# imazen/image-webp

Measured on AMD Instinct MI355X. Metric: 1920x1080 lossy encodes/s (Q75, method 4), higher is better.
Workload: dtype int32; 1 GPU; encode_frame_lossy 1920x1080 RGBA Q75 m4; device_batch=1024, distinct_frames=4, mbs_per_frame=8160, parallelism=frames sharded over 1 GPU(s), steps_pipelined=True, pipeline_lanes=2

## Files before the change

image-webp_amd/csrc/zw_enc_kernels.hip:

```cpp
#include "zw_dev.h"

#include <type_traits>

#include "zw_enc_rows.h"

#ifdef ZW_NW
#define ZW_NW1 ZW_NW
#define ZW_NW2 ZW_NW
#endif
#ifndef ZW_NW1
#define ZW_NW1 12
#endif
#ifndef ZW_NW2
#define ZW_NW2 12
#endif
#define NW_MAX (ZW_NW1 > ZW_NW2 ? ZW_NW1 : ZW_NW2)
#ifndef ZW_DYN_PRIO
#define ZW_DYN_PRIO 1
#endif
#ifndef ZW_DYN_PRIO1
#define ZW_DYN_PRIO1 2
#endif
#ifndef ZW_P1_LUMA_MAX
#define ZW_P1_LUMA_MAX 3
#endif
#ifndef ZW_CHAIN_PRIO
#define ZW_CHAIN_PRIO 3
#endif
#ifndef ZW_LUMA_PRIO
#define ZW_LUMA_PRIO 0
#endif
#ifndef ZW_UVQ_CHAIN_ROWS
#define ZW_UVQ_CHAIN_ROWS 1
#endif
#ifndef ZW_UVQ_CHAIN_BATCH
#define ZW_UVQ_CHAIN_BATCH 0
#endif
#ifndef ZW_PAIR_UNROLL
#define ZW_PAIR_UNROLL 1
#endif
#ifndef ZW_FETCH_AHEAD
#define ZW_FETCH_AHEAD (PASS == 2)
#endif
#ifndef ZW_AN4_GPW
#define ZW_AN4_GPW 1
#endif

template <int PASS> struct PassShape {
    static constexpr int NW = PASS == 1 ? ZW_NW1 : ZW_NW2;
    static constexpr int WG = NW * 64;
};

__device__ __forceinline__ int rgb_y(const uint8_t* p)
{
    return (16839 * p[0] + 33059 * p[1] + 6420 * p[2] + (1 << 15) + (16 << 16)) >> 16;
}
__device__ __forceinline__ int rgb_u(const uint8_t* p) { return -9719 * p[0] - 19081 * p[1] + 28800 * p[2] + (128 << 16); }
// ... 478 lines not shown
        uint32_t t01 = cnt[0] + cnt[1], t23 = cnt[2] + cnt[3];
#define GETP(a, b) ((a) + (b) == 0 ? 255 : (uint8_t)((255 * (a) + ((a) + (b)) / 2) / ((a) + (b))))
        P.seg_probs[0] = GETP(t01, t23);
        P.seg_probs[1] = GETP(cnt[0], cnt[1]);
        P.seg_probs[2] = GETP(cnt[2], cnt[3]);
#undef GETP
        P.seg_update_map = P.seg_probs[0] != 255 || P.seg_probs[1] != 255 || P.seg_probs[2] != 255;
        P.seg_enabled = 1;
    }
    params[f] = P;
    uint4* Hz = (uint4*)(histo + (size_t)f * 256);
    for (int i = 0; i < 64; i++) Hz[i] = make_uint4(0u, 0u, 0u, 0u);
}

struct EncArgs {
    const uint8_t *Y, *U, *V;
    const uint8_t* alpha;
    const ZwFrameParams* params;
    const ZwLevelCosts* lcost;
    int8_t* derr;
    ZwMbOut* out;
    uint8_t *ry, *ru, *rv;
    size_t ysz, csz;
    int mbw, mbh, pass;
    int* dbg;
    uint8_t* rows;
    uint32_t* sizes;
    int nframes;
};

struct MbLds {
    uint8_t sy[256], su[64], sv[64];
    uint8_t ws[17 * ZW_BPS];
    uint8_t left_y[20], left_u[12], left_v[12], left_c[12];
    int8_t left_derr[4];
    uint8_t modes[16];
    int16_t lev[25][16];
};

struct WaveLds {
    MbLds mb;
    uint8_t cu[9 * ZW_BPS], cv[9 * ZW_BPS];
    uint32_t uvc[64][8];
    int dc[64];
    int y2d[64];
    int y2cost[4];
    int V[2][40];
    int nzt[4], nzl[4];
    int misc[16];
    uint32_t pst[2][4];
    uint8_t win_y[32], win_u[8], win_v[8], win_c[12];
    int8_t win_d[4];
#ifdef ZW_PHASE_PROF
    unsigned long long ph[24];
#endif
};


struct Ctx {
    const EncArgs* a;
    const ZwFrameParams* P;
    int method;
    const ZwSegment* S;
    const ZwSegment* Sl;
    const LdsTables* T;
    WaveLds* W;
    MbLds* M;
    uint8_t *top_y, *top_u, *top_v, *top_c;
    int8_t* top_derr;
    const uint8_t *srcY, *srcU, *srcV;
    const uint8_t *sY, *sU, *sV;
    int ys, cs;
    int mbx, mby, lane, seg;
    int f;
    int oy, oc, ocx, od;
};

__device__ void build_luma_border(const Ctx& C, int part = 2)
{
    uint8_t* ws = C.M->ws;
    const int l = C.lane;
    const int mbw = C.a->mbw;
    const bool want = part == 2 || (part == 0 ? (l < 17 || l >= 32) : (l >= 17 && l < 32));
    if (!want) {
    } else if (l < 32) {
        int v;
        if (l == 0) v = C.mby == 0 ? 127 : (C.mbx == 0 ? 129 : C.M->left_y[0]);
        else if (C.mby == 0) v = 127;
        else if (l <= 16) v = C.top_y[C.oy + l - 1];
        else if (C.mbx == mbw - 1) v = C.top_y[C.oy + 15];
        else v = C.top_y[C.oy + l - 1];
        ws[l] = (uint8_t)v;
        if (l >= 17 && l < 21) {
            ws[4 * ZW_BPS + l] = (uint8_t)v;
            ws[8 * ZW_BPS + l] = (uint8_t)v;
            ws[12 * ZW_BPS + l] = (uint8_t)v;
        }
    } else if (l < 48) {
        int i = l - 32;
        ws[(i + 1) * ZW_BPS] = C.mbx == 0 ? 129 : C.M->left_y[1 + i];
    }
    wsync();
}

__device__ void build_chroma_border(const Ctx& C)
{
    const int l = C.lane;
// ... 66 lines not shown
        const int d = wht_g(c[0], b);
        const int t = b > 0;
        const int ay = (int)((__umul24((uint32_t)iabs(d), S.y2.iq[t]) + S.y2.bias[t]) >> 17);
        const int qy = d < 0 ? -ay : ay;
        y2cost = (int)rcost_g<0, PASS == 2>(qy, b, 0, 1, T);
        dq[0] = iwht_g(m24(qy, (int)S.y2.q[t]), b);
    }
    idct16(dq);
    int rec[16], sse = 0, flat = 1;
    const int s00 = C.sY[0];
#pragma unroll
    for (int k = 0; k < 16; k++) {
        rec[k] = clamp255(pr[k] + dq[k]);
        const int d = src[k] - rec[k];
        sse += m24(d, d);
        flat &= src[k] == s00;
    }
    int td = iabs(ttransform_diff_pk(rec, src)) >> 5;
    sse = red16(sse);
    td = red16(td);
    cost = red16(cost);
    nzac = red16(nzac);
    flat = red16(flat);
    const int srcflat = __builtin_amdgcn_readlane(flat, 0) == 16;
    cost += y2cost;
    int sd = S.tlambda > 0 ? ((int)S.tlambda * td + 128) >> 8 : 0;
    int dfin = sse;
    if (srcflat && nzac == 0) {
        dfin = sse * 2;
        sd = sd * 2;
    }
    const int mcost = sel4(m, d_FIXED_COSTS_I16[0], d_FIXED_COSTS_I16[1], d_FIXED_COSTS_I16[2], d_FIXED_COSTS_I16[3]) + cost;
    const int dist = dfin + sd;
    long long brd = 0x7fffffffffffffffLL, bfin = 0;
    int bm = 0;
#pragma unroll
    for (int mm = 0; mm < 4; mm++) {
        const long long mc = __builtin_amdgcn_readlane(mcost, mm * 16);
        const long long dd = 256LL * __builtin_amdgcn_readlane(dist, mm * 16);
        const long long r_m = mc * (long long)S.l_i16 + dd;
        const long long f_m = mc * (long long)S.l_mode + dd;
        const int avail = mm == 0 || (mm == 1 && above) || (mm == 2 && left) || (mm == 3 && above && left);
        if (avail && r_m < brd) {
            brd = r_m;
            bfin = f_m;
            bm = mm;
        }
    }
    best_mode = bm;
    best_score = bfin < 0 ? 0ull : (unsigned long long)bfin;
}

#ifdef ZW_PHASE_PROF
__device__ unsigned long long zw_phase_cycles_dev[2][24];
__device__ unsigned long long zw_wave_cycles_dev[2][16][24];
#define PH_START() long long ph_t_ = clock64()
#define PH_RESET() (ph_t_ = clock64())
#define PH_MARK(k) PH_MARK_L(k, lane, PASS)
#define PH_MARK_L(k, ln, ps)                                                        \
    do {                                                                            \
        const long long n_ = clock64();                                             \
        if ((ln) == 0) C.W->ph[k] += (unsigned long long)(n_ - ph_t_);               \
        ph_t_ = n_;                                                                 \
    } while (0)
extern "C" int zw_wave_cycles(unsigned long long* out, int reset)
{
    if (hipMemcpyFromSymbol(out, HIP_SYMBOL(zw_wave_cycles_dev), sizeof(zw_wave_cycles_dev)) != hipSuccess) return -1;
    if (reset) {
        static unsigned long long z[2][16][24];
        if (hipMemcpyToSymbol(HIP_SYMBOL(zw_wave_cycles_dev), z, sizeof z) != hipSuccess) return -1;
    }
    return 0;
}
extern "C" int zw_phase_cycles(unsigned long long* out, int reset)
{
    if (hipMemcpyFromSymbol(out, HIP_SYMBOL(zw_phase_cycles_dev), sizeof(zw_phase_cycles_dev)) != hipSuccess) return -1;
    if (reset) {
        static unsigned long long z[2][24];
        if (hipMemcpyToSymbol(HIP_SYMBOL(zw_phase_cycles_dev), z, sizeof z) != hipSuccess) return -1;
    }
    return 0;
}
#define PH_COUNT(k) \
    do {                \
        if (C.lane == 0) C.W->ph[k] += 1; \
    } while (0)
#elif defined(ZW_ASM_MARKS)
#define PH_COUNT(k) (void)0
#define PH_START() asm volatile("; ZWMARK start" ::: "memory")
#define PH_RESET() (void)0
#define PH_MARK(k) asm volatile("; ZWMARK " #k ::: "memory")
#define PH_MARK_L(k, ln, ps) asm volatile("; ZWMARK " #k ::: "memory")
#else
#define PH_COUNT(k) (void)0
#define PH_START() (void)0
#define PH_RESET() (void)0
#define PH_MARK(k) (void)0
#define PH_MARK_L(k, ln, ps) (void)0
#endif

template <int NB>
__device__ __forceinline__ void i4_values_n(const Ctx& C, const int* x0, const int* y0)
{
    WaveLds* W = C.W;
    const uint8_t* ws = C.M->ws;
    const int l = C.lane;
    const int t = (int)(l >= 13) + (int)(l >= 24) + (int)(l >= 36) + (int)(l >= 37);
    const int k = min(l - 13 * (int)(l >= 13) - 11 * (int)(l >= 24), 12);
    const int t3 = (int)(t == 3), t4 = (int)(t >= 4), t12 = (int)(t == 1 || t == 2);
    const int ka = k + t3 * (11 - k) + t4 * (1 - k);
    const int kb = k + t12 + t3 * (12 - k) - t4 * k;
    const int kc = min(k + 2 * (int)(t == 1), 12);
    const int wb = 2 * (int)(t == 1) + (int)(t == 2) + 3 * (t3 + t4);
    const int wc = (int)(t == 1);
    const int sh = (int)(t != 0) + (int)(t != 0 && t != 2);
    const int oa = csel(ka < 4, -ka * ZW_BPS, ka - 4 - 4 * ZW_BPS);
    const int ob = csel(kb < 4, -kb * ZW_BPS, kb - 4 - 4 * ZW_BPS);
    const int oc = csel(kc < 4, -kc * ZW_BPS, kc - 4 - 4 * ZW_BPS);
    const bool dcl = l < 4 || (l >= 5 && l < 9);
    int v[NB], ea[NB];
#pragma unroll
    for (int h = 0; h < NB; h++) {
        const int rowL = (y0[h] + 3) * ZW_BPS + x0[h] - 1;
        ea[h] = ws[rowL + oa];
        const int eb = ws[rowL + ob], ec = ws[rowL + oc];
        v[h] = (ea[h] + wb * eb + wc * ec + ((1 << sh) >> 1)) >> sh;
    }
#pragma unroll
    for (int h = 0; h < NB; h++) {
        const int dsum = red16(dcl ? ea[h] : 0);
        if (l < 38) W->V[h][l] = v[h];
// ... 1135 lines not shown
        for (int i = 0; i < 16; i++) {
            const int sby = i >> 2, sbx = i & 3, x0 = sbx * 4 + 1, y0 = sby * 4 + 1;
            const int bm = C.M->modes[i];
            i4_values(C, x0, y0);
            const int k = l & 15;
            const int pk = i4_pred_at(W->V[0], i4_src_index(C.T, bm, k), W->V[0][5 + (k & 3)] - W->V[0][4]);
            const int svk = C.sY[(sby * 4 + (k >> 2)) * 16 + sbx * 4 + (k & 3)];
            const int ck = fdct_g(svk - pk, k);
            const int ctx0 = min(left_nz[sby] + top_nz[sbx], 2);
            if (C.a->dbg && C.a->pass == 2 && l < 16) {
                int* d = C.a->dbg + (((size_t)C.f * C.a->mbw * C.a->mbh + (size_t)C.mby * C.a->mbw + C.mbx) * 16 + i) * 34;
                d[k] = ck;
                d[16 + k] = pk;
                if (k == 0) {
                    d[32] = ctx0;
                    d[33] = bm;
                }
            }
            const int qs = quantz(ck, S.y1.iq[k > 0], S.y1.bias[k > 0]);
            const int snz = gmask(qs != 0) != 0;
            int dqk, nzq;
            if (trel) {
                const int cn = gget(ck, zz_of(k));
                int lvn;
                nzq = trellis_g<0>(cn, k, S.y1, S.sharpen, S.lt_i4, C.T, 3, ctx0, lvn);
                if (l < 16) C.M->lev[i][k] = (int16_t)lvn;
                dqk = m24(gget(lvn, izz_of(k)), (int)S.y1.q[k > 0]);
            } else {
                if (l < 16) C.M->lev[i][izz_of(k)] = (int16_t)qs;
                nzq = snz;
                dqk = m24(qs, (int)S.y1.q[k > 0]);
            }
            const int rk = idct_g(dqk, k);
            if (l < 16) C.M->ws[(y0 + (k >> 2)) * ZW_BPS + x0 + (k & 3)] = (uint8_t)clamp255(pk + rk);
            wsync();
            if (l == 0) {
                W->misc[1] = nzq;
                W->misc[2] = snz;
            }
            wsync();
            const int nz = W->misc[1];
            anynz |= W->misc[2];
            top_nz[sbx] = nz;
            left_nz[sby] = nz;
            y_nz_out[i] = nz;
            wsync();
        }
        if (l < 16) C.M->lev[16][l] = 0;
        wsync();
        PH_MARK_L(15, l, 0);
        PH_COUNT(7);
    }
    return anynz;
}

__device__ int final_chroma(const Ctx& C, int mode, int8_t* top_derr, int uv_nz[8])
{
    WaveLds* W = C.W;
    const ZwSegment& S = *C.S;
    const int l = C.lane;
    const int h = l >> 5, b = l & 7, pl = b >> 2, bx = b & 1, by = (b >> 1) & 1;
    const bool act = (l & 31) < 8;
    int cf[2][4];
    uint32_t p01[2], p32[2];
    {
        const uint32_t* e = W->uvc[h * 32 + mode * 8 + b];
#pragma unroll
        for (int c = 0; c < 2; c++) {
            cf[c][0] = lo16(e[2 * c]);
            cf[c][1] = hi16(e[2 * c]);
            cf[c][2] = lo16(e[2 * c + 1]);
            cf[c][3] = hi16(e[2 * c + 1]);
        }
        p01[0] = e[4];
        p32[0] = e[5];
        p01[1] = e[6];
        p32[1] = e[7];
    }
    {
        const int q = (int)S.uv.q[0];
        const uint32_t iq = S.uv.iq[0], bias = S.uv.bias[0];
        const uint32_t zt = S.uv.zthresh[0];
        int dcs[8];
#pragma unroll
        for (int k = 0; k < 8; k++) dcs[k] = __builtin_amdgcn_readlane(cf[0][0], k);
        auto diffuse = [&](int& dc, int te, int le) -> int {
            dc += (7 * te + 8 * le) >> 3;
            const int sign = dc < 0;
            const uint32_t a = (uint32_t)(sign ? -dc : dc);
            const int level = a > zt ? (int)((a * iq + bias) >> 17) : 0;
            const int err = (int)a - level * q;
            const int se = sign ? -err : err;
            const int v = se >> 1;
            return (int)(int8_t)(v < -127 ? -127 : (v > 127 ? 127 : v));
        };
#pragma unroll
        for (int ch = 0; ch < 2; ch++) {
            int8_t* top = top_derr + ch * 2;
            int8_t* lft = C.M->left_derr + ch * 2;
            const int t0 = __builtin_amdgcn_readfirstlane((int)top[0]), t1 = __builtin_amdgcn_readfirstlane((int)top[1]);
            const int l0 = __builtin_amdgcn_readfirstlane((int)lft[0]), l1 = __builtin_amdgcn_readfirstlane((int)lft[1]);
            int* d = dcs + ch * 4;
            const int e0 = diffuse(d[0], t0, l0);
            const int e1 = diffuse(d[1], t1, e0);
            const int e2 = diffuse(d[2], e0, l1);
            const int e3 = diffuse(d[3], e1, e2);
// ... 554 lines not shown
            (&Tf->lc[0][0][0][0])[i] = a.lcost ? (&a.lcost[ff].lc[0][0][0][0])[i] : 0;
        for (int i = threadIdx.x; i < 96; i += WG) {
            (&Tf->eob[0][0][0])[i] = a.lcost ? (&a.lcost[ff].eob[0][0][0])[i] : 0;
            (&Tf->init[0][0][0])[i] = a.lcost ? (&a.lcost[ff].init[0][0][0])[i] : 0;
        }
        for (int i = threadIdx.x; i < 4 * 8 * 3 * 11; i += WG) (&Tf->probs[0][0][0][0])[i] = (&Pf->probs[0][0][0][0])[i];
        static_assert(sizeof(ZwSegment) % 4 == 0, "segment copy by dwords");
        for (int i = threadIdx.x; i < (int)(4 * sizeof(ZwSegment) / 4); i += WG)
            ((uint32_t*)Sf)[i] = ((const uint32_t*)Pf->seg)[i];
        for (int i = threadIdx.x; i < 256; i += WG) lut[i] = Pf->seg_enabled ? Pf->seg_map_lut[i] : 0;
        load_static_tables(Tf, threadIdx.x, WG, &Pf->probs[0][0][0][0]);
        if (!ROWS || chain_wg) {
            uint8_t* ty = top_y + L.sy * fr;
            uint8_t* tu = top_u + L.su * fr;
            uint8_t* tv = top_v + L.sv * fr;
            uint8_t* tcx = top_c + L.sc * fr;
            int8_t* td = top_derr + L.sd * fr;
            if (!ROWS) {
                for (int i = threadIdx.x; i < mbw * 16 + 48; i += WG) ty[i] = 127;
                for (int i = threadIdx.x; i < mbw * 12; i += WG) tcx[i] = 0;
            }
            for (int i = threadIdx.x; i < mbw * 8 + 48; i += WG) {
                tu[i] = 127;
                tv[i] = 127;
            }
            for (int i = threadIdx.x; i < mbw * 4; i += WG) td[i] = PASS == 2 ? a.derr[(size_t)ff * mbw * 4 + i] : 0;
        }
    }
    if (threadIdx.x < NW) progress[threadIdx.x] = -1;
    if (threadIdx.x < 2) xflag[threadIdx.x] = 0;
    if (ROWS && lane < 12) W->win_c[lane] = 0;
    __syncthreads();

    Ctx C;
    C.a = &a;
    C.P = P;
    C.T = T;
    C.W = W;
    C.M = &W->mb;
    C.lane = lane;
    C.f = f;
    C.Sl = Sl;
    C.method = __builtin_amdgcn_readfirstlane(P->method);
    C.top_y = top_y;
    C.top_u = top_u;
    C.top_v = top_v;
    C.top_c = top_c;
    C.top_derr = top_derr;
    C.oy = C.oc = C.ocx = C.od = 0;
    const bool trel = PASS == 2 && __builtin_amdgcn_readfirstlane(P->do_trellis);
    const bool keep_i4 = !trel && (PASS == 1 || a.dbg == nullptr);
    const size_t nmb = (size_t)mbw * mbh;
#ifdef ZW_PHASE_PROF
    if (lane < 24) W->ph[lane] = 0;
    wsync();
    auto ph_flush = [&]() {
        if (lane < 24) atomicAdd(&zw_phase_cycles_dev[PASS - 1][lane], W->ph[lane]);
        if (lane < 24) atomicAdd(&zw_wave_cycles_dev[PASS - 1][wv][lane], W->ph[lane]);
    };
#else
    auto ph_flush = []() {};
#endif

    if (chain_wg) {
        __builtin_amdgcn_s_setprio(ZW_CHAIN_PRIO);
        const int cfr = PAIR ? wv : 0;
        const bool has_chain = !PAIR || cfr < nf;
        const int fc = f + (has_chain ? cfr : 0);
        const uint8_t* const lutc = seg_lut + L.sL * cfr;
        int8_t* const tdc = top_derr + L.sd * cfr;
        if (PAIR) {
            C.f = fc;
            C.P = a.params + fc;
            C.T = (const LdsTables*)((const uint8_t*)T + L.sT * cfr);
            C.Sl = (const ZwSegment*)((const uint8_t*)Sl + L.sS * cfr);
            C.top_u = top_u + L.su * cfr;
            C.top_v = top_v + L.sv * cfr;
            C.top_derr = tdc;
            C.method = __builtin_amdgcn_readfirstlane(C.P->method);
        }
        if (lane < 4) C.M->left_derr[lane] = 0;
        if (NCH == 2 && !PAIR) {
            const int pl = wv;
            UvQ U;
            U.pl = pl;
            U.w = W->cu;
            U.sp = C.M->su;
            U.top = pl ? top_v : top_u;
            U.left = C.M->left_u;
            const uint8_t* const P0 = (pl ? a.V : a.U) + (size_t)f * a.csz;
            const int cs = mbw * 8;
            auto fetch_uv = [&](int mbx, int mby) {
                MbFetch r;
                r.y = lane < 16 ? *(const uint32_t*)(P0 + (size_t)(mby * 8 + (lane >> 1)) * cs + mbx * 8 + (lane & 1) * 4)
                                : 0u;
                r.c = 0;
                r.alpha = a.alpha[(size_t)f * nmb + (size_t)mby * mbw + mbx];
                return r;
            };
            C.ys = mbw * 16;
            C.cs = cs;
            MbFetch nx = fetch_uv(0, 0);
            int seq = 0;
            for (int mby = 0; mby < mbh; mby++) {
                if (lane < 12) C.M->left_u[lane] = 129;
                wsync();
                for (int mbx = 0; mbx < mbw; mbx++) {
                    PH_START();
                    const int lane = opaque_lane(threadIdx.x & 63);
                    C.lane = lane;
                    const MbFetch cur = nx;
// ... 32 lines not shown
                C.M->left_v[lane] = 129;
            }
            wsync();
            for (int mbx = 0; mbx < mbw; mbx++) {
                PH_START();
                const int lane = opaque_lane(threadIdx.x & 63);
                C.lane = lane;
                const MbFetch cur = nx;
                if (mbx + 1 < mbw) nx = fetch_mb(&a, fc, lane, mbx + 1, mby);
                else if (mby + 1 < mbh) nx = fetch_mb(&a, fc, lane, 0, mby + 1);
                setup_ctx(C, &a, lutc, W, mbx, mby, cur);
                C.oc = mbx * 8;
                C.ocx = mbx * 12;
                build_chroma_border(C);
                const int cm = pick_uv<PASS>(C);
                PH_MARK(8);
                int uvnz[8];
                final_chroma(C, cm, tdc + mbx * 4, uvnz);
                PH_MARK(9);
                store_chroma_borders(C);
                ZwMbOut* o = a.out + (size_t)fc * nmb + (size_t)mby * mbw + mbx;
                if (lane == 0) o->chroma_mode = (uint8_t)cm;
                write_levels(C, 17, 8, false);
                wsync();
            }
        }
        for (int i = lane; has_chain && i < mbw * 4; i += 64) a.derr[(size_t)fc * mbw * 4 + i] = tdc[i];
        if (!PAIR) {
            ph_flush();
            return;
        }
        C.f = f;
        C.P = P;
        C.T = T;
        C.Sl = Sl;
        C.top_u = top_u;
        C.top_v = top_v;
        C.top_derr = top_derr;
        C.method = __builtin_amdgcn_readfirstlane(P->method);
    }

    if (PASS == 1) __builtin_amdgcn_s_setprio(ZW_LUMA_PRIO);
    using RS = RowSchedule<PASS, ROWS, NW, NCH>;
    constexpr bool skip_mode = RS::skip_mode;
    constexpr int nrw = RS::nrw;
    const int rw = ROWS ? 0 : RS::first_row(wv, mbh);
    if (ROWS) {
        C.top_y = W->win_y;
        C.top_u = W->win_u;
        C.top_v = W->win_v;
        C.top_c = W->win_c;
        C.top_derr = W->win_d;
    }
    auto mb_store = [&](Ctx& C, int lm, int cm, bool i4reuse, uint32_t i4nz, bool trel) __attribute__((always_inline)) {
        const int lane = C.lane;
        PH_START();
        int ynz[16];
        const int lnz = final_luma(C, lm, trel, ynz, i4reuse ? (int)i4nz : -1);
        PH_MARK(4);
        int uvnz[8] = {0, 0, 0, 0, 0, 0, 0, 0};
        int cnz = 0;
        if (PASS == 2) cnz = final_chroma(C, cm, C.top_derr + C.od, uvnz);
        PH_MARK(5);
        ZwMbOut* o = a.out + (size_t)C.f * nmb + (size_t)C.mby * mbw + C.mbx;
        if (PASS == 2) {
            const int skip = !(lnz | cnz);
            if (lane == 0) {
                uint8_t* tc = C.top_c + C.ocx;
                uint8_t* lc = C.M->left_c;
                if (skip) {
                    for (int k = 1; k < 9; k++) tc[k] = lc[k] = 0;
                    if (lm != 4) tc[0] = lc[0] = 0;
                } else {
                    if (lm != 4) {
                        int y2nz = 0;
                        for (int n = 0; n < 16; n++) y2nz |= C.M->lev[16][n] != 0;
                        tc[0] = lc[0] = (uint8_t)y2nz;
                    }
                    for (int x = 0; x < 4; x++) tc[1 + x] = (uint8_t)ynz[12 + x];
                    for (int y = 0; y < 4; y++) lc[1 + y] = (uint8_t)ynz[y * 4 + 3];
                    tc[5] = (uint8_t)uvnz[2];
                    tc[6] = (uint8_t)uvnz[3];
                    lc[5] = (uint8_t)uvnz[1];
                    lc[6] = (uint8_t)uvnz[3];
                    tc[7] = (uint8_t)uvnz[6];
                    tc[8] = (uint8_t)uvnz[7];
                    lc[7] = (uint8_t)uvnz[5];
                    lc[8] = (uint8_t)uvnz[7];
                }
                o->skip = (uint8_t)skip;
                o->chroma_mode = (uint8_t)cm;
            }
            store_chroma_borders(C);
            write_levels(C, 0, 25, skip);
            if (a.sizes) {
                int e = 0;
                if (lane < 25 && !skip) {
                    const uint32_t* lw = (const uint32_t*)C.M->lev[lane];
#pragma unroll
                    for (int q = 0; q < 8; q++) {
                        const uint32_t v = lw[q];
                        e = (v >> 16) ? 2 * q + 2 : ((v & 0xffffu) ? 2 * q + 1 : e);
                    }
                }
                const int r16 = red16(e);
                const int es = __builtin_amdgcn_readlane(r16, 0) + __builtin_amdgcn_readlane(r16, 16);
                if (lane == 0)
                    a.sizes[(size_t)C.f * nmb + (size_t)C.mby * mbw + C.mbx] = (uint32_t)(1 + (lm == 4 ? 8 : 0) + 25 + 2 * es);
            }
        } else {
            write_levels(C, 0, 17, false);
            if (lane == 0) o->skip = 0;
        }
        if (lane == 0) {
            o->luma_mode = (uint8_t)lm;
            o->segment = (uint8_t)C.seg;
        }
        if (lane < 16) o->bpred[lane] = lm == 4 ? C.M->modes[lane] : 0;
        store_luma_borders(C);
    };
    if constexpr (PAIR) {
        MbLds* const Mp[2] = {&W->mb, Mall2 + wv};
        const int meth0 = C.method;
        const int K = C.method <= 3 ? 3 : (C.method == 4 ? 4 : 10);
        const int meth1 = nf == 2 ? __builtin_amdgcn_readfirstlane(a.params[f + 1].method) : C.method;
        const bool trel1 = PASS == 2 && nf == 2 && __builtin_amdgcn_readfirstlane(a.params[f + 1].do_trellis);
        const bool keep1 = !trel1 && (PASS == 1 || a.dbg == nullptr);
        using RP =
            typename std::conditional<PASS == 1, PairRowSchedule1<NW, NCW>, RowSchedule<PASS, ROWS, NW, NCW, true>>::type;
        const bool same_k = nf == 1 || (meth1 == C.method && trel1 == trel);
        for (int mby = RP::first_row(wv, mbh); mby < mbh; mby = RP::next_row(wv, mby, mbh)) {
#pragma unroll
            for (int fr = 0; fr < 2; fr++) row_start(Mp[fr], lane);
            wsync();
            const int prevw = mby > 0 ? RP::wave_of_row(mby - 1, mbh) : 0;
            auto wait_above = [&](int need) {
                if (mby > 0) wait_row(progress, prevw, (mby - 1) * 65536 + need);
            };
            for (int mbx = 0; mbx < mbw; mbx++) {
                PH_START();
                const int lane = opaque_lane(threadIdx.x & 63);
                C.lane = lane;
                auto enter = [&](int fr) {
                    C.lane = opaque_lane(threadIdx.x & 63);
                    C.f = f + fr;
                    C.P = a.params + C.f;
                    C.T = (const LdsTables*)((const uint8_t*)T + L.sT * fr);
                    C.Sl = (const ZwSegment*)((const uint8_t*)Sl + L.sS * fr);
                    C.top_y = top_y + L.sy * fr;
                    C.top_u = top_u + L.su * fr;
                    C.top_v = top_v + L.sv * fr;
                    C.top_c = top_c + L.sc * fr;
                    C.top_derr = top_derr + L.sd * fr;
                    C.M = fr ? Mp[1] : Mp[0];
                    C.method = fr ? meth1 : meth0;
                    C.mbx = mbx;
                    C.mby = mby;
                    C.oy = mbx * 16;
                    C.oc = mbx * 8;
                    C.ocx = mbx * 12;
                    C.od = mbx * 4;
                    C.sY = C.M->sy;
                    C.sU = C.M->su;
                    C.sV = C.M->sv;
                };
                auto pst = [&](int fr, int k) { return (uint32_t)__builtin_amdgcn_readfirstlane((int)W->pst[fr][k]); };
                wait_above(min(mbx + 1, mbw));
                luma_issue_prio<PASS>(progress, prevw, mbx, mby, mbw);
                PH_MARK(0);
ZW_PAIR_LOOP
                for (int fr = 0; fr < 2; fr++) {
                    if (fr >= nf) {
// ... 13 lines not shown
                        W->pst[fr][1] = (uint32_t)s_;
                        W->pst[fr][2] = (uint32_t)(s_ >> 32);
                        W->pst[fr][3] = 0;
                    }
                    wsync();
                }
                wsync();
                PH_MARK(1);
                const uint32_t s0 = pst(0, 0), s1 = pst(1, 0);
                const bool n0 = (s0 >> 4) & 1u, n1 = (s1 >> 4) & 1u;
                if (n0 || n1) wait_above(min(mbx + 2, mbw));
ZW_PAIR_LOOP
                for (int fr = 0; fr < 2; fr++) {
                    if (!((pst(fr, 0) >> 4) & 1u)) continue;
                    enter(fr);
                    build_luma_border(C, 1);
                }
                PH_MARK(21);
                if (K <= 4 && same_k && (n0 || n1)) {
                    Ctx CA = C, CB = C;
                    CA.lane = CB.lane = opaque_lane(threadIdx.x & 63);
                    CA.T = T;
                    CB.T = (const LdsTables*)((const uint8_t*)T + L.sT);
                    CA.M = Mp[0];
                    CB.M = Mp[1];
                    CA.S = Sl + (s0 >> 8);
                    CB.S = (const ZwSegment*)((const uint8_t*)Sl + L.sS) + (s1 >> 8);
                    CA.sY = Mp[0]->sy;
                    CB.sY = Mp[1]->sy;
                    const unsigned long long i0 = pst(0, 1) | ((unsigned long long)pst(0, 2) << 32);
                    const unsigned long long i1 = pst(1, 1) | ((unsigned long long)pst(1, 2) << 32);
                    uint32_t z0 = 0, z1 = 0;
                    const uint32_t r = pick_i4_pair<PASS>(CA, CB, i0, i1, n0, n1, keep_i4, z0, z1);
                    if (lane == 0) {
                        W->pst[0][3] = (r & 1u) ? (z0 | 0x10000u) : 0u;
                        W->pst[1][3] = (r & 2u) ? (z1 | 0x10000u) : 0u;
                    }
                } else if (n0 || n1) {
ZW_PAIR_LOOP
                    for (int fr = 0; fr < 2; fr++) {
                        const uint32_t sm = pst(fr, 0);
                        if (!((sm >> 4) & 1u)) continue;
                        enter(fr);
                        C.seg = (int)(sm >> 8);
                        C.S = C.Sl + C.seg;
                        uint32_t z = 0;
                        const bool w4 = pick_i4<PASS>(C, pst(fr, 1) | ((unsigned long long)pst(fr, 2) << 32),
                                                      fr ? keep1 : keep_i4, z);
                        if (lane == 0) W->pst[fr][3] = w4 ? (z | 0x10000u) : 0u;
                    }
                }
                wsync();
                PH_MARK(2);
ZW_PAIR_LOOP
                for (int fr = 0; fr < 2; fr++) {
                    if (fr >= nf) continue;
                    enter(fr);
                    const uint32_t sm = pst(fr, 0), r4 = pst(fr, 3);
                    C.seg = (int)(sm >> 8);
                    C.S = C.Sl + C.seg;
                    int cm = 0;
                    if (PASS == 2) {
                        build_chroma_border(C);
                        cm = pick_uv<PASS>(C);
                    }
                    PH_MARK(3);
                    const bool w4 = (r4 >> 16) & 1u;
                    mb_store(C, w4 ? 4 : (int)(sm & 15u), cm, w4 && (fr ? keep1 : keep_i4), r4 & 0xffffu,
                             fr ? trel1 : trel);
                    PH_RESET();
                }
                publish(progress, wv, mby * 65536 + mbx + 1);
                PH_MARK(6);
            }
        }
        ph_flush();
        return;
    }
    uint8_t* const gty = ROWS ? rb + RL.ty : nullptr;
    uint8_t* const gtu = ROWS ? rb + RL.tu : nullptr;
    uint8_t* const gtv = ROWS ? rb + RL.tv : nullptr;
    uint8_t* const gtc = ROWS ? rb + RL.tc : nullptr;
    uint8_t* const gtd = ROWS ? rb + RL.td : nullptr;
    for (int it = 0, yk = rw;; it++) {
        const int mby = ROWS ? row_ticket(&rsync[0]) : (skip_mode ? yk : rw + it * nrw);
        if (skip_mode) yk = RS::next_row(wv, yk, mbh);
        if (mby >= mbh) break;
        row_start(C.M, lane);
        wsync();
        const int prevw = (!ROWS && mby > 0) ? RS::wave_of_row(mby - 1) : 0;
        int seen = -1;
        int* const prog_above = ROWS ? rsync + 4 + (mby > 0 ? mby - 1 : 0) : nullptr;
        auto wait_above = [&](int need) {
            if (mby == 0) return;
            if (ROWS) row_wait(prog_above, need, rerr, seen);
            else wait_row(progress, prevw, (mby - 1) * 65536 + need);
        };
        MbFetch nx;
        if (ZW_FETCH_AHEAD) nx = fetch_mb(&a, f, lane, 0, mby);
        for (int mbx = 0; mbx < mbw; mbx++) {
            PH_START();
            const int lane = opaque_lane(threadIdx.x & 63);
            C.lane = lane;
            MbFetch cur;
            if (ZW_FETCH_AHEAD) {
                cur = nx;
                if (mbx + 1 < mbw) nx = fetch_mb(&a, f, lane, mbx + 1, mby);
            } else {
                cur = fetch_mb(&a, f, lane, mbx, mby);
            }
            wait_above(min(mbx + 1, mbw));
            if (ROWS) {
                if (mby > 0) {
                    uint32_t v = 0;
                    if (lane < 4) v = ld_sc1(gty + mbx * 16 + 4 * lane);
                    else if (PASS == 2 && lane < 6) v = ld_sc1(gtu + mbx * 8 + 4 * (lane - 4));
                    else if (PASS == 2 && lane < 8) v = ld_sc1(gtv + mbx * 8 + 4 * (lane - 6));
                    else if (PASS == 2 && lane < 11) v = ld_sc1(gtc + mbx * 12 + 4 * (lane - 8));
                    else if (PASS == 2 && lane < 12) v = ld_sc1(gtd + mbx * 4);
                    if (lane < 4) ((uint32_t*)W->win_y)[lane] = v;
                    else if (PASS == 2 && lane < 6) ((uint32_t*)W->win_u)[lane - 4] = v;
                    else if (PASS == 2 && lane < 8) ((uint32_t*)W->win_v)[lane - 6] = v;
                    else if (PASS == 2 && lane < 11) ((uint32_t*)W->win_c)[lane - 8] = v;
                    else if (PASS == 2 && lane < 12) ((uint32_t*)W->win_d)[0] = v;
// ... 298 lines not shown
```

Measured before the change: 4468 encodes/s.

## Encode luma of both paired frames in one wave pass with compacted trellis tasks

In the paired-frame path, the final luma reconstruction for i16 macroblocks of both frames runs together in a single 64-lane wave pass: lanes 0-15 handle frame A's 4x4 blocks and lanes 32-47 handle frame B's. For trellis, blocks that quantize trivially to zero are found up front. Only the needed (block, context) trellis tasks are then compacted onto lanes, so both frames usually share one speculative trellis call and the context chain is resolved afterwards. Chroma is moved ahead of luma and its results are stashed in LDS, and per-MB output is split into luma, chroma and finish steps. The aim is to cut the serial per-frame luma cost and idle lanes, at the price of more complex code and speculative trellis over multiple contexts.

```diff
diff --git a/image-webp_amd/csrc/zw_enc_kernels.hip b/image-webp_amd/csrc/zw_enc_kernels.hip
--- a/image-webp_amd/csrc/zw_enc_kernels.hip
+++ b/image-webp_amd/csrc/zw_enc_kernels.hip
@@ -3,6 +3,9 @@
 #include <type_traits>
 
 #include "zw_enc_rows.h"
+#include "zw_enc_pairfinal.h"
+
+#define ZW_PH_N 28
 
 #ifdef ZW_NW
 #define ZW_NW1 ZW_NW
@@ -587,7 +590,7 @@
     uint8_t win_y[32], win_u[8], win_v[8], win_c[12];
     int8_t win_d[4];
 #ifdef ZW_PHASE_PROF
-    unsigned long long ph[24];
+    unsigned long long ph[ZW_PH_N];
 #endif
 };
 
@@ -760,8 +763,8 @@
 }
 
 #ifdef ZW_PHASE_PROF
-__device__ unsigned long long zw_phase_cycles_dev[2][24];
-__device__ unsigned long long zw_wave_cycles_dev[2][16][24];
+__device__ unsigned long long zw_phase_cycles_dev[2][ZW_PH_N];
+__device__ unsigned long long zw_wave_cycles_dev[2][16][ZW_PH_N];
 #define PH_START() long long ph_t_ = clock64()
 #define PH_RESET() (ph_t_ = clock64())
 #define PH_MARK(k) PH_MARK_L(k, lane, PASS)
@@ -775,7 +778,7 @@
 {
     if (hipMemcpyFromSymbol(out, HIP_SYMBOL(zw_wave_cycles_dev), sizeof(zw_wave_cycles_dev)) != hipSuccess) return -1;
     if (reset) {
-        static unsigned long long z[2][16][24];
+        static unsigned long long z[2][16][ZW_PH_N];
         if (hipMemcpyToSymbol(HIP_SYMBOL(zw_wave_cycles_dev), z, sizeof z) != hipSuccess) return -1;
     }
     return 0;
@@ -784,7 +787,7 @@
 {
     if (hipMemcpyFromSymbol(out, HIP_SYMBOL(zw_phase_cycles_dev), sizeof(zw_phase_cycles_dev)) != hipSuccess) return -1;
     if (reset) {
-        static unsigned long long z[2][24];
+        static unsigned long long z[2][ZW_PH_N];
         if (hipMemcpyToSymbol(HIP_SYMBOL(zw_phase_cycles_dev), z, sizeof z) != hipSuccess) return -1;
     }
     return 0;
@@ -2026,6 +2029,211 @@
         PH_COUNT(7);
     }
     return anynz;
+}
+
+__device__ void final_luma_pair(const Ctx& CA, const Ctx& CB, int modeA, int modeB, bool trel, uint32_t& resA,
+                                uint32_t& resB)
+{
+    [[maybe_unused]] const Ctx& C = CA;
+    WaveLds* W = CA.W;
+    const int l = CA.lane, hm = l >> 5, b = l & 15, bx = b & 3, by = b >> 2;
+    const bool own = (l & 16) == 0;
+    PH_START();
+    build_luma_border(CA);
+    build_luma_border(CB);
+    MbLds* const M = hm ? CB.M : CA.M;
+    const ZwSegment* const S = hm ? CB.S : CA.S;
+    const uint8_t* const sY = hm ? CB.sY : CA.sY;
+    const int mode = hm ? modeB : modeA;
+    const uint8_t* ws = M->ws;
+    const int above = CA.mby != 0, left = CA.mbx != 0;
+    int dcv;
+    {
+        const int v = (int)ws[csel(own, 1 + b, (b + 1) * ZW_BPS)] & -(int)(own ? above : left);
+        const int sum = red16(v);
+        const int sa = __builtin_amdgcn_readlane(sum, 0) + __builtin_amdgcn_readlane(sum, 16);
+        const int sb = __builtin_amdgcn_readlane(sum, 32) + __builtin_amdgcn_readlane(sum, 48);
+        const int shf = 3 + above + left;
+        dcv = (!above && !left) ? 128 : (((hm ? sb : sa) + (1 << (shf - 1))) >> shf);
+    }
+    int c[16];
+    uint32_t ppk[4];
+    {
+        const int P0 = ws[0];
+        int L[4], Tp[4], r[16];
+#pragma unroll
+        for (int i = 0; i < 4; i++) {
+            L[i] = ws[(by * 4 + i + 1) * ZW_BPS];
+            Tp[i] = ws[1 + bx * 4 + i];
+        }
+#pragma unroll
+        for (int i = 0; i < 4; i++) {
+            const uint32_t srow = *(const uint32_t*)(sY + (by * 4 + i) * 16 + bx * 4);
+            ppk[i] = 0;
+#pragma unroll
+            for (int j = 0; j < 4; j++) {
+                const int p = sel4(mode, dcv, Tp[j], L[i], clamp255(L[i] + Tp[j] - P0));
+                ppk[i] |= (uint32_t)p << (8 * j);
+                r[i * 4 + j] = (int)((srow >> (8 * j)) & 255u) - p;
+            }
+        }
+        fdct16_pk(r, c);
+    }
+    int y2dq;
+    uint32_t anyA, anyB;
+    {
+        const int d = wht_g(c[0], b);
+        const int t = b > 0;
+        const int y2q = quantz(d, S->y2.iq[t], S->y2.bias[t]);
+        if (own) M->lev[16][izz_of(b)] = (int16_t)y2q;
+        y2dq = iwht_g(m24(y2q, (int)S->y2.q[t]), b);
+        int snz = y2q != 0;
+        const uint32_t iq1 = S->y1.iq[1], bs1 = S->y1.bias[1];
+#pragma unroll
+        for (int k = 1; k < 16; k++) snz |= quantz(c[k], iq1, bs1) != 0;
+        const unsigned long long any = __ballot(snz != 0);
+        anyA = (uint32_t)any != 0u;
+        anyB = (uint32_t)(any >> 32) != 0u;
+    }
+    PH_MARK_L(16, l, 0);
+    const int q1 = (int)S->y1.q[1];
+    int nzb = 0;
+    auto finish = [&](bool act, int* lv) {
+        wsync();
+        if (act) {
+            int dq[16];
+            lv[0] = 0;
+#pragma unroll
+            for (int n = 0; n < 16; n++) M->lev[b][n] = (int16_t)lv[n];
+#pragma unroll
+            for (int n = 1; n < 16; n++) dq[kZZ(n)] = m24(lv[n], q1);
+            dq[0] = y2dq;
+            idct16(dq);
+            uint8_t* wsp = M->ws;
+#pragma unroll
+            for (int k = 0; k < 16; k++) {
+                const int y = by * 4 + (k >> 2), x = bx * 4 + (k & 3);
+                const int p = (int)((ppk[k >> 2] >> (8 * (k & 3))) & 255u);
+                wsp[(y + 1) * ZW_BPS + 1 + x] = (uint8_t)clamp255(p + dq[k]);
+            }
+        }
+    };
+    if (trel) {
+        const bool tzl = pf_trivial(c, (uint32_t)q1, S->y1.iq[1], S->sharpen);
+        const unsigned long long tzb = __ballot(tzl);
+        const unsigned tzA = (unsigned)tzb & 0xffffu, tzB = (unsigned)(tzb >> 32) & 0xffffu;
+        unsigned eA = 0, eB = 0;
+#pragma unroll
+        for (int q = 0; q < 4; q++) {
+            eA |= (unsigned)(__builtin_amdgcn_readfirstlane(CA.top_c[CA.ocx + 1 + q]) != 0) << q;
+            eA |= (unsigned)(__builtin_amdgcn_readfirstlane(CA.M->left_c[1 + q]) != 0) << (4 + q);
+            eB |= (unsigned)(__builtin_amdgcn_readfirstlane(CB.top_c[CB.ocx + 1 + q]) != 0) << q;
+            eB |= (unsigned)(__builtin_amdgcn_readfirstlane(CB.M->left_c[1 + q]) != 0) << (4 + q);
+        }
+        unsigned long long mA = 0, mB = 0;
+        {
+            const unsigned need = pf_need(b, hm ? tzB : tzA, hm ? eB : eA);
+#pragma unroll
+            for (int cx = 0; cx < 3; cx++) {
+                const unsigned long long nb = __ballot((need >> cx) & 1u);
+                mA |= (nb & 0xffffull) << (16 * cx);
+                mB |= ((nb >> 32) & 0xffffull) << (16 * cx);
+            }
+        }
+        const bool one = pf_one_call(mA, mB);
+        if (own) {
+            uint32_t* st = (uint32_t*)M->lev[b];
+#pragma unroll
+            for (int i = 0; i < 8; i++) st[i] = pack_lo(c[2 * i], c[2 * i + 1]);
+        }
+        if (one) PH_COUNT(24);
+        else PH_COUNT(25);
+        const int ncall = one ? 1 : 2;
+#pragma nounroll
+        for (int r = 0; r < ncall; r++) {
+            const unsigned long long cA = one ? mA : (r == 0 ? ZW_PF_ALL : 0ull);
+            const unsigned long long cB = one ? mB : (r == 1 ? ZW_PF_ALL : 0ull);
+            const int nA = pf_count(cA), nT = nA + pf_count(cB);
+            const unsigned long long cm = hm ? cB : cA;
+            const int base = hm ? nA : 0;
+            if (own) {
+#pragma unroll
+                for (int cx = 0; cx < 3; cx++)
+                    if ((cm >> (cx * 16 + b)) & 1ull) W->dc[pf_task(cm, base, b, cx) & 63] = (hm << 6) | (cx << 4) | b;
+            }
+            wsync();
+            int lv[16];
+#pragma unroll
+            for (int n = 0; n < 16; n++) lv[n] = 0;
+            int tnz = 0;
+            if (l < nT) {
+                const int td = W->dc[l];
+                const bool tf = (td >> 6) & 1;
+                const ZwSegment* const St = tf ? CB.S : CA.S;
+                const uint32_t* st = (const uint32_t*)(tf ? CB.M : CA.M)->lev[td & 15];
+                int dq[16];
+#pragma unroll
+                for (int i = 0; i < 8; i++) {
+                    const uint32_t w = st[i];
+                    dq[2 * i] = lo16(w);
+                    dq[2 * i + 1] = hi16(w);
+                }
+                tnz = trellis<1, true>(dq, lv, St->y1, St->sharpen, St->lt_i16, tf ? CB.T : CA.T, 0, (td >> 4) & 3);
+            }
+            PH_MARK_L(17, l, 0);
+            const unsigned long long nzm = __ballot(l < nT && tnz);
+            auto chain = [&](unsigned long long cmf, int basef, unsigned tz, unsigned e, unsigned& code,
+                             unsigned& nzbits) {
+                int nt[4], nl[4];
+#pragma unroll
+                for (int q = 0; q < 4; q++) {
+                    nt[q] = (int)((e >> q) & 1u);
+                    nl[q] = (int)((e >> (4 + q)) & 1u);
+                }
+                code = nzbits = 0;
+#pragma unroll
+                for (int bb = 0; bb < 16; bb++) {
+                    const int cx = min(nl[bb >> 2] + nt[bb & 3], 2);
+                    const int z = ((tz >> bb) & 1u) ? 0 : (int)((nzm >> (pf_task(cmf, basef, bb, cx) & 63)) & 1ull);
+                    nt[bb & 3] = z;
+                    nl[bb >> 2] = z;
+                    code |= (unsigned)cx << (2 * bb);
+                    nzbits |= (unsigned)z << bb;
+                }
+            };
+            unsigned codeA = 0, nzA = 0, codeB = 0, nzB = 0;
+            if (one || r == 0) chain(cA, 0, tzA, eA, codeA, nzA);
+            if (one || r == 1) chain(cB, nA, tzB, eB, codeB, nzB);
+            const int cxb = (int)(((hm ? codeB : codeA) >> (2 * b)) & 3u);
+            const int srcl = pf_task(cm, base, b, cxb) & 63;
+            const bool act = own && (one || r == hm);
+            const bool zero = (((hm ? tzB : tzA) >> b) & 1u) != 0u;
+            int gl[16];
+#pragma unroll
+            for (int i = 0; i < 8; i++) {
+                const uint32_t w = (uint32_t)__shfl((int)pack_lo(lv[2 * i], lv[2 * i + 1]), srcl);
+                gl[2 * i] = zero ? 0 : lo16(w);
+                gl[2 * i + 1] = zero ? 0 : hi16(w);
+            }
+            if (act) nzb = (int)(((hm ? nzB : nzA) >> b) & 1u);
+            PH_MARK_L(18, l, 0);
+            finish(act, gl);
+            wsync();
+        }
+    } else {
+        int lv[16];
+#pragma unroll
+        for (int n = 1; n < 16; n++) {
+            lv[n] = quantz(c[kZZ(n)], S->y1.iq[1], S->y1.bias[1]);
+            nzb |= lv[n] != 0;
+        }
+        finish(own, lv);
+    }
+    const unsigned long long nzall = __ballot(own && nzb);
+    resA = ((uint32_t)nzall & 0xffffu) | (anyA << 16);
+    resB = ((uint32_t)(nzall >> 32) & 0xffffu) | (anyB << 16);
+    wsync();
+    PH_MARK_L(14, l, 0);
 }
 
 __device__ int final_chroma(const Ctx& C, int mode, int8_t* top_derr, int uv_nz[8])
@@ -2686,11 +2894,11 @@
     const bool keep_i4 = !trel && (PASS == 1 || a.dbg == nullptr);
     const size_t nmb = (size_t)mbw * mbh;
 #ifdef ZW_PHASE_PROF
-    if (lane < 24) W->ph[lane] = 0;
+    if (lane < ZW_PH_N) W->ph[lane] = 0;
     wsync();
     auto ph_flush = [&]() {
-        if (lane < 24) atomicAdd(&zw_phase_cycles_dev[PASS - 1][lane], W->ph[lane]);
-        if (lane < 24) atomicAdd(&zw_wave_cycles_dev[PASS - 1][wv][lane], W->ph[lane]);
+        if (lane < ZW_PH_N) atomicAdd(&zw_phase_cycles_dev[PASS - 1][lane], W->ph[lane]);
+        if (lane < ZW_PH_N) atomicAdd(&zw_wave_cycles_dev[PASS - 1][wv][lane], W->ph[lane]);
     };
 #else
     auto ph_flush = []() {};
@@ -2829,16 +3037,29 @@
         C.top_c = W->win_c;
         C.top_derr = W->win_d;
     }
-    auto mb_store = [&](Ctx& C, int lm, int cm, bool i4reuse, uint32_t i4nz, bool trel) __attribute__((always_inline)) {
+    auto mb_luma = [&](Ctx& C, int lm, bool i4reuse, uint32_t i4nz, bool trel) __attribute__((always_inline)) {
+        int ynz[16];
+        uint32_t r = (uint32_t)(final_luma(C, lm, trel, ynz, i4reuse ? (int)i4nz : -1) != 0) << 16;
+#pragma unroll
+        for (int k = 0; k < 16; k++) r |= (uint32_t)(ynz[k] != 0) << k;
+        return r;
+    };
+    auto mb_chroma = [&](Ctx& C, int cm) __attribute__((always_inline)) {
+        int uvnz[8];
+        uint32_t r = (uint32_t)(final_chroma(C, cm, C.top_derr + C.od, uvnz) != 0) << 8;
+#pragma unroll
+        for (int k = 0; k < 8; k++) r |= (uint32_t)(uvnz[k] != 0) << k;
+        return r;
+    };
+    auto mb_finish = [&](Ctx& C, int lm, int cm, uint32_t lres, uint32_t cres, bool chroma_borders)
+                         __attribute__((always_inline)) {
         const int lane = C.lane;
-        PH_START();
-        int ynz[16];
-        const int lnz = final_luma(C, lm, trel, ynz, i4reuse ? (int)i4nz : -1);
-        PH_MARK(4);
-        int uvnz[8] = {0, 0, 0, 0, 0, 0, 0, 0};
-        int cnz = 0;
-        if (PASS == 2) cnz = final_chroma(C, cm, C.top_derr + C.od, uvnz);
-        PH_MARK(5);
+        int ynz[16], uvnz[8];
+#pragma unroll
+        for (int k = 0; k < 16; k++) ynz[k] = (int)((lres >> k) & 1u);
+#pragma unroll
+        for (int k = 0; k < 8; k++) uvnz[k] = (int)((cres >> k) & 1u);
+        const int lnz = (int)((lres >> 16) & 1u), cnz = (int)((cres >> 8) & 1u);
         ZwMbOut* o = a.out + (size_t)C.f * nmb + (size_t)C.mby * mbw + C.mbx;
         if (PASS == 2) {
             const int skip = !(lnz | cnz);
@@ -2868,7 +3089,7 @@
                 o->skip = (uint8_t)skip;
                 o->chroma_mode = (uint8_t)cm;
             }
-            store_chroma_borders(C);
+            if (chroma_borders) store_chroma_borders(C);
             write_levels(C, 0, 25, skip);
             if (a.sizes) {
                 int e = 0;
@@ -2895,6 +3116,15 @@
         }
         if (lane < 16) o->bpred[lane] = lm == 4 ? C.M->modes[lane] : 0;
         store_luma_borders(C);
+    };
+    auto mb_store = [&](Ctx& C, int lm, int cm, bool i4reuse, uint32_t i4nz, bool trel) __attribute__((always_inline)) {
+        [[maybe_unused]] const int lane = C.lane;
+        PH_START();
+        const uint32_t lres = mb_luma(C, lm, i4reuse, i4nz, trel);
+        PH_MARK(4);
+        const uint32_t cres = PASS == 2 ? mb_chroma(C, cm) : 0u;
+        PH_MARK(5);
+        mb_finish(C, lm, cm, lres, cres, true);
     };
     if constexpr (PAIR) {
         MbLds* const Mp[2] = {&W->mb, Mall2 + wv};
@@ -3014,24 +3244,79 @@
                 }
                 wsync();
                 PH_MARK(2);
+                if (PASS == 2) {
+ZW_PAIR_LOOP
+                    for (int fr = 0; fr < 2; fr++) {
+                        if (fr >= nf) continue;
+                        enter(fr);
+                        C.seg = (int)(pst(fr, 0) >> 8);
+                        C.S = C.Sl + C.seg;
+                        build_chroma_border(C);
+                        const int cm = pick_uv<PASS>(C);
+                        PH_MARK(3);
+                        const uint32_t cres = mb_chroma(C, cm);
+                        store_chroma_borders(C);
+                        if (lane == 0) W->pst[fr][1] = cres | ((uint32_t)cm << 9);
+                        PH_MARK(5);
+                    }
+                }
+                const uint32_t w0 = pst(0, 3), w1 = pst(1, 3);
+                if (nf == 2 && !((w0 | w1) & 0x10000u) && trel == trel1) {
+                    Ctx CA = C, CB = C;
+                    CA.lane = CB.lane = opaque_lane(threadIdx.x & 63);
+                    CA.f = f;
+                    CB.f = f + 1;
+                    CA.T = T;
+                    CB.T = (const LdsTables*)((const uint8_t*)T + L.sT);
+                    CA.M = Mp[0];
+                    CB.M = Mp[1];
+                    CA.S = Sl + (s0 >> 8);
+                    CB.S = (const ZwSegment*)((const uint8_t*)Sl + L.sS) + (s1 >> 8);
+                    CA.sY = Mp[0]->sy;
+                    CB.sY = Mp[1]->sy;
+                    CA.top_y = top_y;
+                    CB.top_y = top_y + L.sy;
+                    CA.top_c = top_c;
+                    CB.top_c = top_c + L.sc;
+                    CA.mbx = CB.mbx = mbx;
+                    CA.mby = CB.mby = mby;
+                    CA.oy = CB.oy = mbx * 16;
+                    CA.ocx = CB.ocx = mbx * 12;
+                    uint32_t r0, r1;
+                    final_luma_pair(CA, CB, (int)(s0 & 15u), (int)(s1 & 15u), trel, r0, r1);
+                    if (lane == 0) {
+                        W->pst[0][2] = r0;
+                        W->pst[1][2] = r1;
+                    }
+                } else {
+ZW_PAIR_LOOP
+                    for (int fr = 0; fr < 2; fr++) {
+                        if (fr >= nf) continue;
+                        enter(fr);
+                        const uint32_t sm = pst(fr, 0), r4 = pst(fr, 3);
+                        C.seg = (int)(sm >> 8);
+                        C.S = C.Sl + C.seg;
+                        const bool w4 = (r4 >> 16) & 1u;
+                        const uint32_t lres = mb_luma(C, w4 ? 4 : (int)(sm & 15u), w4 && (fr ? keep1 : keep_i4),
+                                                      r4 & 0xffffu, fr ? trel1 : trel);
+                        if (lane == 0) W->pst[fr][2] = lres;
+                    }
+                    if (nf == 2) PH_COUNT(26);
+                }
+                wsync();
+                PH_MARK(4);
 ZW_PAIR_LOOP
                 for (int fr = 0; fr < 2; fr++) {
                     if (fr >= nf) continue;
                     enter(fr);
-                    const uint32_t sm = pst(fr, 0), r4 = pst(fr, 3);
+                    const uint32_t sm = pst(fr, 0), r4 = pst(fr, 3), cr = pst(fr, 1);
                     C.seg = (int)(sm >> 8);
                     C.S = C.Sl + C.seg;
-                    int cm = 0;
-                    if (PASS == 2) {
-                        build_chroma_border(C);
-                        cm = pick_uv<PASS>(C);
-                    }
-                    PH_MARK(3);
                     const bool w4 = (r4 >> 16) & 1u;
-                    mb_store(C, w4 ? 4 : (int)(sm & 15u), cm, w4 && (fr ? keep1 : keep_i4), r4 & 0xffffu,
-                             fr ? trel1 : trel);
-                    PH_RESET();
+                    mb_finish(C, w4 ? 4 : (int)(sm & 15u), PASS == 2 ? (int)(cr >> 9) : 0, pst(fr, 2),
+                              PASS == 2 ? cr & 0x1ffu : 0u, false);
                 }
+                PH_RESET();
                 publish(progress, wv, mby * 65536 + mbx + 1);
                 PH_MARK(6);
             }
diff --git a/image-webp_amd/csrc/zw_enc_pairfinal.h b/image-webp_amd/csrc/zw_enc_pairfinal.h
--- /dev/null
+++ b/image-webp_amd/csrc/zw_enc_pairfinal.h
@@ -0,0 +1,85 @@
+#pragma once
+#include <stdint.h>
+
+#ifndef ZW_HD
+#ifdef __HIPCC__
+#define ZW_HD __host__ __device__
+#else
+#define ZW_HD
+#endif
+#endif
+
+#if defined(__HIP_DEVICE_COMPILE__)
+#define ZW_PF_UMUL(a, b) __umul24((a), (b))
+#define ZW_PF_POPC(v) __popcll(v)
+#else
+#define ZW_PF_UMUL(a, b) ((uint32_t)(a) * (uint32_t)(b))
+#define ZW_PF_POPC(v) __builtin_popcountll(v)
+#endif
+
+#define ZW_PF_MAX_TASKS 40
+#define ZW_PF_LANES 64
+
+ZW_HD inline int pf_zz(int n) { return (int)((0xfeb7adc963258410ull >> (4 * n)) & 15); }
+
+ZW_HD inline bool pf_trivial(const int* c, uint32_t q_ac, uint32_t iq_ac, const uint16_t* sharpen)
+{
+    const uint32_t thresh = ZW_PF_UMUL(q_ac, q_ac) / 4u;
+    const uint32_t tbias = ((0x80u << 17) + 128u) >> 8;
+    int last = 0;
+    uint32_t live = 0;
+    for (int n = 1; n < 16; n++) {
+        const int j = pf_zz(n);
+        const uint32_t a = (uint32_t)(c[j] < 0 ? -c[j] : c[j]);
+        if (ZW_PF_UMUL(a, a) > thresh) last = n;
+        const uint32_t thr = (ZW_PF_UMUL(a + sharpen[j], iq_ac) + tbias) >> 17;
+        live |= (uint32_t)(thr != 0u) << n;
+    }
+    if (last < 15) last++;
+    return (live & ((2u << last) - 1u)) == 0u;
+}
+
+ZW_HD inline unsigned pf_edge(const int* top4, const int* left4)
+{
+    unsigned e = 0;
+    for (int q = 0; q < 4; q++) e |= ((unsigned)(top4[q] != 0) << q) | ((unsigned)(left4[q] != 0) << (4 + q));
+    return e;
+}
+
+ZW_HD inline unsigned pf_need(int b, unsigned triv, unsigned edge)
+{
+    const int bx = b & 3, by = b >> 2;
+    const unsigned lt = (triv >> ((b - 1) & 15)) & 1u, tt = (triv >> ((b - 4) & 15)) & 1u;
+    const unsigned kl = bx == 0 ? (edge >> (4 + by)) & 1u : 0u, ul = bx == 0 ? 0u : lt ^ 1u;
+    const unsigned kt = by == 0 ? (edge >> bx) & 1u : 0u, ut = by == 0 ? 0u : tt ^ 1u;
+    const unsigned k = kl + kt, u = ul + ut;
+    const unsigned run = (1u << (k + u + 1u)) - (1u << k);
+    return ((triv >> b) & 1u) ? 0u : run;
+}
+
+ZW_HD inline uint64_t pf_mask(unsigned triv, unsigned edge)
+{
+    uint64_t m = 0;
+    for (int b = 0; b < 16; b++) {
+        const unsigned nd = pf_need(b, triv, edge);
+        for (int cx = 0; cx < 3; cx++) m |= (uint64_t)((nd >> cx) & 1u) << (cx * 16 + b);
+    }
+    return m;
+}
+
+ZW_HD inline int pf_count(uint64_t mask) { return (int)ZW_PF_POPC(mask); }
+
+ZW_HD inline int pf_task(uint64_t mask, int base, int b, int cx)
+{
+    return base + (int)ZW_PF_POPC(mask & ((1ull << (cx * 16 + b)) - 1ull));
+}
+
+#ifndef ZW_PF_COMPACT
+#define ZW_PF_COMPACT 1
+#endif
+ZW_HD inline bool pf_one_call(uint64_t mask_a, uint64_t mask_b)
+{
+    return ZW_PF_COMPACT && pf_count(mask_a) + pf_count(mask_b) <= ZW_PF_LANES;
+}
+
+#define ZW_PF_ALL 0xffffffffffffull
```

New measurement: 4615 encodes/s (median of 6 runs). +3.3%, better.
